# PlakarLabs/plakar

Hardware: AMD Instinct MI355X
Metric: GiB/s chunked (device-resident, cut-points out) at 1/2/4/8 MI355X (higher is better)
Workload: dtype u8; 1 GPU; C1: 1x 1 GiB uniform random buffer per GPU (BASELINE configs[1]); bytes_per_gpu=1073741824, global_bytes=1073741824, buffers_per_gpu=1, chunk_params=FASTCDC min 65536 / normal 1048576 / max 4194304, gear=placeholder (v0.0.8 table unavailable; see DESIGN.md), parallelism=independent buffers, 1 rank per GPU x 1, no collective, streams=2

## Files before the change

plakar_amd/csrc/cdc_kernels.hip:

```cpp
#include <hip/hip_ext.h>
#include <hip/hip_runtime.h>

#include <algorithm>
#include <mutex>
#include <type_traits>
#include <vector>

#include "cdc_hostmem.h"
#include "cdc_internal.h"

namespace cdc {

#ifndef CDC_SPIN_SLEEP
#define CDC_SPIN_SLEEP 1
#endif
constexpr int kSpinSleep = CDC_SPIN_SLEEP;

static constexpr uint64_t kNoHit = ~0ull;
static constexpr uint32_t kRawLaneBytes = 512;
static constexpr uint32_t kWarm = 64;

template <int NT, int COPIES = 32>
__device__ __forceinline__ void fill_gear_lds(uint64_t *tab, const uint64_t *gear, uint32_t sh = 0)
{
    static_assert(NT % 64 == 0, "block size");
    constexpr uint32_t kSlots = 256u * COPIES;
    constexpr int kPer = int((kSlots + NT - 1) / NT);
    uint64_t v[kPer];
#pragma unroll
    for (int i = 0; i < kPer; ++i) {
        const uint32_t x = threadIdx.x + uint32_t(i) * NT;
        v[i] = x < kSlots ? gear[x / COPIES] : 0;
    }
#pragma unroll
    for (int i = 0; i < kPer; ++i) {
        const uint32_t x = threadIdx.x + uint32_t(i) * NT;
        if (x < kSlots) tab[x] = v[i] << sh;
    }
}
constexpr uint32_t kWCopies = 8;
constexpr uint32_t kWEntShift = kWCopies == 32 ? 8 : kWCopies == 16 ? 7 : 6;
static_assert(kWCopies == 8 || kWCopies == 16 || kWCopies == 32, "walker table copies");

__device__ __forceinline__ uint64_t lds_gear(const char *tab, uint32_t addr)
{
    return *reinterpret_cast<const uint64_t *>(tab + addr);
}

typedef __attribute__((address_space(3))) const char lds_char;
typedef __attribute__((address_space(1))) const uint64_t g_u64;
typedef __attribute__((address_space(1))) const uint32_t g_u32;
typedef __attribute__((address_space(1))) const uint8_t g_u8;

__device__ __forceinline__ uint64_t lds_gear(const lds_char *tab, uint32_t addr)
{
    return *reinterpret_cast<__attribute__((address_space(3))) const uint64_t *>(tab + addr);
}

template <typename T>
__device__ __forceinline__ T *as_space(uint64_t addr)
{
    return reinterpret_cast<T *>(uintptr_t(addr));
}

__device__ __forceinline__ const lds_char *as_lds(const char *p)
{
    return as_space<const lds_char>(uint32_t(reinterpret_cast<uintptr_t>(p)));
}

__device__ __forceinline__ uint4 gload16(uint64_t a)
{
    const g_u64 *q = as_space<const g_u64>(a);
    const uint64_t x = q[0], y = q[1];
    return make_uint4(uint32_t(x), uint32_t(x >> 32), uint32_t(y), uint32_t(y >> 32));
}

__device__ __forceinline__ uint32_t gear_addr(uint32_t laneoff, uint32_t word, int k)
{
    return __builtin_amdgcn_perm(laneoff, word, 0x0C0C0004u | (uint32_t(k & 3) << 8));
}

template <uint32_t ESH = kWEntShift>
__device__ __forceinline__ uint32_t wgear_addr(uint32_t wlaneoff, uint32_t word, int k)
{
    if constexpr (ESH == 8) return gear_addr(wlaneoff, word, k);
    return (__builtin_amdgcn_ubfe(word, uint32_t(k & 3) * 8u, 8u) << ESH) | wlaneoff;
}

__device__ __forceinline__ uint32_t key_of(uint64_t fp, uint32_t mlo, uint32_t mhi)
{
    return __builtin_amdgcn_bitop3_b32(uint32_t(fp >> 32), mhi, uint32_t(fp) & mlo, 0xEA);
}

__device__ __forceinline__ uint32_t word_of(const uint4 &d, int i)
{
    return i == 0 ? d.x : i == 1 ? d.y : i == 2 ? d.z : d.w;
}

__device__ __forceinline__ uint32_t umin3(uint32_t a, uint32_t b, uint32_t c)
{
    uint32_t r;
    asm("v_min3_u32 %0, %1, %2, %3" : "=v"(r) : "v"(a), "v"(b), "v"(c));
    return r;
}

template <uint32_t ESH = kWEntShift, typename TP>
__device__ __forceinline__ uint32_t roll16_test(const uint4 &d, uint64_t &fp, TP tab,
                                                uint32_t laneoff, uint32_t mlo, uint32_t mhi)
{
    uint32_t acc = 0xFFFFFFFFu;
#pragma unroll
    for (int k = 0; k < 16; ++k) {
        fp = (fp << 1) + lds_gear(tab, wgear_addr<ESH>(laneoff, word_of(d, k >> 2), k));
        acc = min(acc, key_of(fp, mlo, mhi));
    }
    return acc;
}

template <uint32_t ESH = kWEntShift, typename TP>
__device__ __forceinline__ void roll16(const uint4 &d, uint64_t &fp, TP tab,
                                       uint32_t laneoff)
{
#pragma unroll
    for (int k = 0; k < 16; ++k)
        fp = (fp << 1) + lds_gear(tab, wgear_addr<ESH>(laneoff, word_of(d, k >> 2), k));
}

template <uint32_t ESH = kWEntShift, typename TP>
__device__ __forceinline__ uint64_t group_first_hit(const uint4 &d, uint64_t &fp, uint64_t a,
                                                    uint64_t ts, uint64_t te, uint64_t fz,
                                                    TP tab, uint32_t laneoff,
                                                    uint32_t mlo, uint32_t mhi)
{
    uint64_t hit = kNoHit;
#pragma unroll
    for (int k = 0; k < 16; ++k) {
        const uint64_t pos = a + k;
        const uint64_t g = lds_gear(tab, wgear_addr<ESH>(laneoff, word_of(d, k >> 2), k));
        fp = pos < fz ? 0ull : (fp << 1) + g;
        if (hit == kNoHit && pos >= ts && pos < te && pos >= fz && key_of(fp, mlo, mhi) == 0)
            hit = pos;
    }
    return hit;
}


__device__ __forceinline__ uint32_t to_vgpr(uint32_t x)
{
    uint32_t v;
    asm volatile("v_mov_b32 %0, %1" : "=v"(v) : "s"(x));
    return v;
}

constexpr uint32_t kDbgTs = 16;
constexpr uint32_t kDbgGraph = 32;
constexpr uint32_t kTsScan = 0;
constexpr uint32_t kTsRes = kTsScan + 4 * 4096;
constexpr uint32_t kTsClk = kTsRes + 8 * 16384;
constexpr uint32_t kClkRecs = 4096;
constexpr uint32_t kTsClkN = kTsClk + 4 * kClkRecs;
constexpr uint32_t kTsHw = kTsClkN + 1;
constexpr uint32_t kTsAbort = kTsHw + 4096;
constexpr uint32_t kTsSlots = kTsAbort + 4;
constexpr uint32_t kDbgClk = 64;
__device__ uint64_t g_ts[kTsSlots];

__device__ __forceinline__ void dbg_ts(const Batch &B, uint32_t slot, uint64_t v = ~0ull)
{
    if ((B.debug & kDbgTs) && slot < kTsSlots) g_ts[slot] = v == ~0ull ? __builtin_amdgcn_s_memrealtime() : v;
}

constexpr uint32_t kAbortWord = kMaxBufsPerLaunch;
constexpr uint32_t kLimitWord = kMaxBufsPerLaunch + 1;
constexpr uint64_t kSpinLimit = 200000000ull;
enum : uint32_t { kWaitJunction = 2, kWaitPrev, kWaitLook, kWaitLookSlow, kWaitLast };

struct SpinGuard {
    uint64_t t0 = 0, lim = 0;
    __device__ __forceinline__ bool ok(uint32_t *flags, uint32_t kind, uint64_t a, uint64_t b)
    {
        const uint64_t now = __builtin_amdgcn_s_memrealtime();
        if (!t0) {
            t0 = now;
            lim = __hip_atomic_load(flags + kLimitWord, __ATOMIC_RELAXED, __HIP_MEMORY_SCOPE_AGENT);
            if (!lim) lim = kSpinLimit;
            return true;
        }
        if (__hip_atomic_load(flags + kAbortWord, __ATOMIC_RELAXED, __HIP_MEMORY_SCOPE_AGENT)) return false;
        if (now - t0 < lim) return true;
        if ((threadIdx.x & 63u) == 0) {
            __hip_atomic_store(flags + kAbortWord, kind, __ATOMIC_RELAXED, __HIP_MEMORY_SCOPE_AGENT);
            g_ts[kTsAbort] = kind;
            g_ts[kTsAbort + 1] = a;
            g_ts[kTsAbort + 2] = b;
            g_ts[kTsAbort + 3] = now;
        }
        return false;
    }
};


#ifndef CDC_SCAN_WAVES
#define CDC_SCAN_WAVES 12
#endif
constexpr uint32_t kS2Waves = CDC_SCAN_WAVES;
constexpr uint32_t kStage = 64;
constexpr uint32_t kL = kStage / 16;
constexpr uint32_t kGroups = kStage / 16;
constexpr uint32_t kStageBytes = 64u * kStage;
constexpr uint32_t kGearLdsBytes = 256u * 32u * 8u;
constexpr uint32_t kQCap = 64;
constexpr uint32_t kQBytes = kQCap * 12u;
constexpr uint32_t kFlushTabBytes = 256u * 8u;
static_assert(kGearLdsBytes + kS2Waves * (kStageBytes + kQBytes) + kFlushTabBytes + 37128u <= 160u * 1024u,
              "LDS budget: a scan workgroup and a k_resolve workgroup per CU");
constexpr uint32_t kLaneQuant = 256;

template <int N>
__device__ __forceinline__ void wait_vmcnt()
{
    static_assert(N == 0, "vmcnt");
    asm volatile("s_waitcnt vmcnt(0)" ::: "memory");
}

#ifdef CDC_SCAN_DMA_DEFAULT_POLICY
#define DMA_PIECE(i) "global_load_lds_dwordx4 %" #i ", %[base]\n\t"
#else
#define DMA_PIECE(i) "global_load_lds_dwordx4 %" #i ", %[base] nt\n\t"
#endif
#define DMA_NEXT "s_add_u32 m0, m0, 0x400\n\ts_nop 0\n\t"
__device__ __forceinline__ void dma_stage(uint64_t base_in, uint32_t dst_in, const uint32_t (&off)[kL])
{
    static_assert(kL == 4, "four 1-KiB pieces per stage");
    const uint64_t base = (uint64_t(uint32_t(__builtin_amdgcn_readfirstlane(uint32_t(base_in >> 32)))) << 32) |
                          uint32_t(__builtin_amdgcn_readfirstlane(uint32_t(base_in)));
    const uint32_t dst = __builtin_amdgcn_readfirstlane(dst_in);
    uint32_t keep;
    asm volatile("s_nop 4\n\ts_mov_b32 %[keep], m0\n\ts_mov_b32 m0, %[dst]\n\ts_nop 0\n\t"
                 DMA_PIECE(1) DMA_NEXT DMA_PIECE(2) DMA_NEXT DMA_PIECE(3) DMA_NEXT DMA_PIECE(4)
                 "s_mov_b32 m0, %[keep]\n\ts_nop 1"
                 : [keep] "=&s"(keep)
                 : "v"(off[0]), "v"(off[1]), "v"(off[2]), "v"(off[3]), [base] "s"(base), [dst] "s"(dst)
                 : "memory", "scc");
}

#ifdef CDC_SCAN_DMA_DEFAULT_POLICY
#define DMA_PIECE_IMM(i, o) "global_load_lds_dwordx4 %" #i ", %[base] offset:" #o "\n\t"
#else
#define DMA_PIECE_IMM(i, o) "global_load_lds_dwordx4 %" #i ", %[base] offset:" #o " nt\n\t"
#endif
__device__ __forceinline__ void dma_stage_imm(uint64_t base_in, uint32_t dst_in, const uint32_t (&offi)[kL])
{
    static_assert(kL == 4, "four 1-KiB pieces per stage");
    const uint64_t base = (uint64_t(uint32_t(__builtin_amdgcn_readfirstlane(uint32_t(base_in >> 32)))) << 32) |
                          uint32_t(__builtin_amdgcn_readfirstlane(uint32_t(base_in)));
    const uint32_t dst = __builtin_amdgcn_readfirstlane(dst_in);
    uint32_t keep;
    asm volatile("s_nop 4\n\ts_mov_b32 %[keep], m0\n\ts_mov_b32 m0, %[dst]\n\ts_nop 0\n\t"
                 DMA_PIECE_IMM(1, 0) DMA_PIECE_IMM(2, 1024) DMA_PIECE_IMM(3, 2048) DMA_PIECE_IMM(4, 3072)
                 "s_mov_b32 m0, %[keep]\n\ts_nop 1"
                 : [keep] "=&s"(keep)
                 : "v"(offi[0]), "v"(offi[1]), "v"(offi[2]), "v"(offi[3]), [base] "s"(base), [dst] "s"(dst)
                 : "memory");
}

__device__ __forceinline__ uint32_t wave_ticket(uint32_t *p)
{
    const uint32_t old = __hip_atomic_fetch_add(p, (threadIdx.x & 63u) == 0u ? 1u : 0u, __ATOMIC_RELAXED,
                                                __HIP_MEMORY_SCOPE_AGENT);
    return __builtin_amdgcn_readfirstlane(old);
}

__device__ __forceinline__ uint32_t scan_wave_max(uint32_t v)
{
#pragma unroll
    for (int o = 32; o; o >>= 1) v = max(v, uint32_t(__shfl_xor(int(v), o)));
    return __builtin_amdgcn_readfirstlane(v);
}

__device__ __forceinline__ uint32_t rec_cnt(uint64_t rec) { return uint32_t(rec & ((1u << kRecCntBits) - 1)); }
__device__ __forceinline__ uint32_t rec_ent(uint64_t rec, uint32_t e)
{
    return uint32_t(rec >> (kRecCntBits + kRecEntBits * e)) & ((1u << kRecEntBits) - 1);
}

__device__ __forceinline__ void record_hit(uint64_t &rec, int32_t r)
{
    const uint32_t c = rec_cnt(rec);
    if (c < kRunCap) rec |= uint64_t(uint32_t(r)) << (kRecCntBits + kRecEntBits * c);
    if (c < (1u << kRecCntBits) - 1) ++rec;
}

constexpr uint64_t kMaskLSpill = 16;

__device__ bool maskl_needed(const Batch &B, const DevParams &P, const Workspace &W, const BufDesc &D, uint64_t t,
                             uint32_t lane)
{
    const uint64_t sl = B.scan_lane, tb = 64ull * sl;
    const uint64_t start = t * tb, end = min(D.len, start + tb);
    const uint64_t ra = start / sl, rb = (end - 1) / sl;
    const uint64_t gap = P.normal_size - P.min_size - (P.win - 1);
    const uint32_t kc = uint32_t(gap / sl > 2 ? gap / sl - 1 : 1);
    const uint64_t r_lo = ra > kc + kMaskLSpill ? ra - kc - kMaskLSpill : 0;
    const uint64_t *runs = W.runs + 64ull * D.task_base;
    uint32_t cur = 0;
    for (uint64_t r4 = r_lo; r4 <= rb; r4 += 256) {
        uint64_t rec[4];
#pragma unroll
        for (int j = 0; j < 4; ++j) {
            const uint64_t q = r4 + 64u * j + lane;
            rec[j] = q <= rb ? runs[q] : 1ull;
        }
#pragma unroll
        for (int j = 0; j < 4; ++j) {
            const uint64_t r0 = r4 + 64u * j;
            if (r0 > rb) break;
            const uint64_t E = __ballot(rec_cnt(rec[j]) == 0);
            const uint32_t n = uint32_t(min(rb + 1 - r0, uint64_t(64)));
            const uint64_t Z = ~E & (n == 64 ? ~0ull : (1ull << n) - 1);
            const uint64_t below = Z & ((1ull << lane) - 1);
            const uint32_t prev = below ? lane - 1u - (63u - uint32_t(__builtin_clzll(below))) : cur + lane;
            const uint64_t r = r0 + lane;
            bool need = false;
            if (lane < n) {
                if ((E >> lane) & 1ull)
                    need = r >= ra && prev + 1 >= kc;
                else
                    need = prev >= kc && r + kMaskLSpill >= ra;
            }
            if (__ballot(need)) return true;
            cur = Z ? n - 1u - (63u - uint32_t(__builtin_clzll(Z))) : cur + n;
        }
    }
    return false;
}

template <bool kMaskL, bool kFused>
__device__ __forceinline__ void scan_task(const Batch &B, const DevParams &P, const Workspace &W, char *s_lds,
                                          const char *tab, uint32_t task, uint32_t lane, uint32_t wave,
                                          uint32_t laneoff);

template <bool kMaskL, bool kFused = false>
__device__ __forceinline__ void scan_body(const Batch &B, const DevParams &P, const Workspace &W)
{
    static_assert(!(kMaskL && kFused), "k_scan_f builds both indexes, from the MaskS records' side");
    __shared__ __attribute__((aligned(16)))
    char s_lds[kGearLdsBytes + kS2Waves * (kStageBytes + kQBytes) + (kFused ? kFlushTabBytes : 0u)];
    const uint32_t lane = threadIdx.x & 63u;
    const uint32_t wave = __builtin_amdgcn_readfirstlane(threadIdx.x >> 6);
    const uint32_t laneoff = (lane & 31u) << 3;
    const uint32_t task = blockIdx.x * kS2Waves + wave;
    bool act = true;
    if constexpr (kMaskL) {
        act = false;
        if (task < B.total_tasks) {
            uint32_t bb = 0;
            while (bb + 1 < B.nbufs && task >= B.b[bb + 1].task_base) ++bb;
            const BufDesc &Db = B.b[bb];
            const uint64_t t = task - Db.task_base;
            if (t * 64ull * B.scan_lane < Db.len) act = maskl_needed(B, P, W, Db, t, lane);
            if (lane == 0) W.validL[task] = act ? 1u : 0u;
        }
        if (!__syncthreads_or(act ? 1 : 0)) return;
        if (threadIdx.x == 0 && B.maskl_hint)
            __hip_atomic_store(B.maskl_hint, 1u, __ATOMIC_RELAXED, __HIP_MEMORY_SCOPE_SYSTEM);
    }
    if constexpr (!kMaskL) {
        const uint32_t gt = blockIdx.x * blockDim.x + threadIdx.x, nth = gridDim.x * blockDim.x;
        for (uint32_t i = gt; i < B.total_segs; i += nth) {
            W.xg[i] = 0ull;
            W.sg[i] = 0ull;
        }
        if (gt < kMaxBufsPerLaunch + 4)
            W.flags[gt] = gt == kLimitWord ? uint32_t(B.spin_ticks ? B.spin_ticks : kSpinLimit) : 0u;
        if (gt < 2) W.tick[gt] = 0u;
        if (gt < B.nbufs) B.b[gt].res->status = kRowPending;
        if (threadIdx.x == 0) dbg_ts(B, kTsScan + 4 * blockIdx.x);
    }
    uint32_t clk = 0;
    if (!kMaskL && (B.debug & kDbgClk) && blockIdx.x == 0 && threadIdx.x == 0) {
        clk = kTsClk + 4u * uint32_t(atomicAdd(reinterpret_cast<unsigned long long *>(&g_ts[kTsClkN]), 1ull) % kClkRecs);
        g_ts[clk] = __builtin_amdgcn_s_memrealtime();
        g_ts[clk + 1] = __builtin_amdgcn_s_memtime();
    }
    fill_gear_lds<kS2Waves * 64>(reinterpret_cast<uint64_t *>(s_lds), W.gear,
                                 kFused ? P.fm_sh : kMaskL ? P.fl_sh : P.fs_sh);
    if constexpr (kFused) {
        static_assert(kS2Waves * 64 >= 256, "one entry per thread");
        if (threadIdx.x < 256)
            reinterpret_cast<uint64_t *>(s_lds + kGearLdsBytes + kS2Waves * (kStageBytes + kQBytes))[threadIdx.x] =
                W.gear[threadIdx.x] << P.fs_sh;
    }
    __syncthreads();
    if (!kMaskL && threadIdx.x == 0) {
        dbg_ts(B, kTsScan + 4 * blockIdx.x + 1);
        if (blockIdx.x < 4096)
            dbg_ts(B, kTsHw + blockIdx.x,
                   uint64_t(__builtin_amdgcn_s_getreg(20 | (0 << 6) | (15 << 11))) << 32 |
                       uint32_t(__builtin_amdgcn_s_getreg(4 | (0 << 6) | (31 << 11))));
    }
    const char *tab = s_lds;
    if (!act) return;
    const bool persist = !kMaskL && B.persist != 0;
    auto next_task = [&]() { return wave_ticket(W.tick + 2); };
    for (uint32_t cur = persist ? next_task() : task;;) {
        if (cur >= B.total_tasks) break;
        scan_task<kMaskL, kFused>(B, P, W, s_lds, tab, cur, lane, wave, laneoff);
        if (!persist) break;
        cur = next_task();
    }
    if (clk && threadIdx.x == 0) {
        g_ts[clk + 2] = __builtin_amdgcn_s_memrealtime();
        g_ts[clk + 3] = __builtin_amdgcn_s_memtime();
    }
}

template <bool kMaskL, bool kFused>
__device__ __forceinline__ void scan_task(const Batch &B, const DevParams &P, const Workspace &W, char *s_lds,
                                          const char *tab, uint32_t task, uint32_t lane, uint32_t wave,
                                          uint32_t laneoff)
{
    uint32_t b = 0;
    while (b + 1 < B.nbufs && task >= B.b[b + 1].task_base) ++b;
    const BufDesc &D = B.b[b];

    const uint64_t sl = B.scan_lane;
    const uint64_t ub = reinterpret_cast<uint64_t>(D.data);
    const uint64_t lo_ok = ub & ~15ull, hi_ok = (ub + D.len + 15) & ~15ull;
    const uint64_t seg0 = uint64_t(task - D.task_base) * 64u;
    if (seg0 * sl >= D.len) return;
    const int64_t s = int64_t((seg0 + lane) * sl);
    constexpr uint32_t kLead = 128u;
    const uint32_t T = uint32_t((sl + kLead + (ub & 15u) + kStage - 1u) / kStage);
    const uint64_t wb = ((ub + seg0 * sl) & ~15ull) - kLead;
    const uint64_t base = wb > lo_ok ? wb : lo_ok;
    const uint64_t limw = hi_ok - 16u - base;
    const uint32_t lim = limw > 0x7FFFFFFFull ? 0x7FFFFFFFu : uint32_t(limw);
    const uint32_t ring = uint32_t(reinterpret_cast<uintptr_t>(s_lds)) + kGearLdsBytes + wave * kStageBytes;
    static_assert(kStage == 64 && kL == 4, "pair staging: 64-B stages, one slot");
    const uint32_t half = lane >> 5;
    const uint32_t row = lane & 31u, swz = (row >> 1) & 7u;
    uint32_t offi[4];
    uint32_t om = 0;
#pragma unroll
    for (uint32_t j = 0; j < 4; ++j) {
        const uint32_t r = 8u * j + lane / 8u;
        const uint32_t k = (lane % 8u) ^ ((r >> 1) & 7u);
        const uint32_t o = uint32_t((((ub + (seg0 + r) * sl) & ~15ull) - kLead + 16u * k) - base);
        om = max(om, o);
        offi[j] = o - 1024u * j;
    }
    const uint64_t om0 = scan_wave_max(om);
    const uint64_t half_step = 32ull * sl;
    auto issue = [&](auto PC, uint32_t u, auto FC) {
        constexpr uint32_t Q = decltype(PC)::value;
        constexpr bool kFast = decltype(FC)::value;
        const uint64_t adv = uint64_t(kStage) * (u - Q) + (Q ? half_step : 0ull);
#ifdef CDC_DIAG_NO_DMA
        return;
#endif
        if (kFast || om0 + adv <= uint64_t(lim)) {
#ifdef CDC_DIAG_L2
            dma_stage_imm(lo_ok + ((base + adv - lo_ok) & 0x7FFF0ull), ring, offi);
#else
            dma_stage_imm(base + adv, ring, offi);
#endif
        } else {
            uint32_t eff[4];
#pragma unroll
            for (uint32_t j = 0; j < 4; ++j) eff[j] = min(offi[j] + 1024u * j + uint32_t(adv), lim);
            dma_stage(base, ring, eff);
        }
    };
    const char *rowp = s_lds + kGearLdsBytes + wave * kStageBytes + row * 128u;
    auto load_row = [&](uint4 (&first)[4], uint4 (&second)[4]) {
#ifdef CDC_DIAG_NO_ROW
        asm volatile("" : "+v"(first[0].x), "+v"(second[0].x));
        return;
#endif
#pragma unroll
        for (uint32_t g = 0; g < 4; ++g) first[g] = *reinterpret_cast<const uint4 *>(rowp + 16u * (g ^ swz));
#pragma unroll
        for (uint32_t g = 0; g < 4; ++g) second[g] = *reinterpret_cast<const uint4 *>(rowp + 16u * ((g + 4) ^ swz));
    };
    const uint32_t TT = T + 1;
    const int32_t lag = int32_t(kStage * half);
    const uint32_t vhi = to_vgpr(kFused ? P.fm_mi : kMaskL ? P.fl_hi : P.fs_hi);
    const uint32_t xlo = kMaskL ? P.fl_lo : P.fs_lo, xhi = kMaskL ? P.fl_hi : P.fs_hi;
    const int64_t rel0 = int64_t(((ub + uint64_t(s)) & ~15ull) - kLead) - int64_t(ub);
    using C0 = std::integral_constant<uint32_t, 0>;
    using C1 = std::integral_constant<uint32_t, 1>;
    using Gen = std::integral_constant<bool, false>;
    using Steady = std::integral_constant<bool, true>;

    uint4 A[4] = {}, Bv[4] = {};
#ifdef CDC_DIAG_WAITS
    uint64_t wsum = 0;
    uint32_t nrc = 0;
    const uint64_t tk0 = __builtin_amdgcn_s_memtime();
    const uint64_t rt0 = __builtin_amdgcn_s_memrealtime();
#endif
    static_assert(kLead >= 2 * kStage, "stage 0 must be pure warm-up for both halves");
    issue(C0{}, 0, Gen{});
    wait_vmcnt<0>();
    if (half == 0) load_row(A, Bv);
    asm volatile("s_waitcnt lgkmcnt(0)" ::: "memory");
    if (1 < TT) issue(C1{}, 1, Gen{});
    if (1 < TT) {
        wait_vmcnt<0>();
        if (half == 1) load_row(Bv, A);
        asm volatile("s_waitcnt lgkmcnt(0)" ::: "memory");
        if (2 < TT) issue(C0{}, 2, Gen{});
    }
    uint64_t gv[2][16];
#pragma unroll
    for (int k = 0; k < 16; ++k) gv[0][k] = lds_gear(tab, gear_addr(laneoff, word_of(Bv[0], k >> 2), k));
    uint64_t fp = 0;
    uint64_t rec = 0;
    uint64_t recL = 0;
    const int32_t rr0 = int32_t(rel0 - s) - lag;
    uint64_t *const qf = reinterpret_cast<uint64_t *>(s_lds + kGearLdsBytes + kS2Waves * kStageBytes + wave * kQBytes);
    uint32_t *const qm = reinterpret_cast<uint32_t *>(qf + kQCap);
    static_assert(kQCap == 64, "one flush pass: item j in lane j");
    uint32_t qn = 0;
    const char *const ftab = s_lds + kGearLdsBytes + kS2Waves * (kStageBytes + kQBytes);
    auto rgear = [&](const uint4 &d, int k) -> uint64_t {
        if constexpr (kFused)
            return lds_gear(ftab, __builtin_amdgcn_ubfe(word_of(d, k >> 2), uint32_t(k & 3) * 8u, 8u) << 3);
        else
            return lds_gear(tab, gear_addr(laneoff, word_of(d, k >> 2), k));
    };
    auto flush = [&]() {
        {
            const bool v = lane < qn;
            const uint32_t meta = qm[v ? lane : 0u];
            const uint32_t owner = meta >> 24;
            const int32_t r0 = int32_t(meta & 0xFFFFFFu) - 256;
            const int64_t so = int64_t((seg0 + owner) * sl);
            const int32_t ln = so < int64_t(D.len) ? int32_t(min(int64_t(sl), int64_t(D.len) - so)) : 0;
            const uint64_t a = ub + uint64_t(so + r0);
            auto clamp16 = [&](uint64_t x) { return min(max(x, lo_ok), hi_ok - 16u); };
            const uint4 d0 = gload16(clamp16(a)), d1 = gload16(clamp16(a + 16u));
            uint64_t f = 0;
            if constexpr (kFused) {
                uint4 dw[4];
#pragma unroll
                for (int h = 0; h < 4; ++h) dw[h] = gload16(clamp16(a - 64u + 16u * uint32_t(h)));
#pragma unroll
                for (int k = 0; k < 64; ++k) f = (f << 1) + rgear(dw[k >> 4], k & 15);
            } else {
                f = qf[v ? lane : 0u];
            }
            uint32_t miss = 0, missL = 0;
#pragma unroll
            for (int k = 0; k < 32; ++k) {
                f = (f << 1) + rgear(k < 16 ? d0 : d1, k & 15);
                miss |= min(key_of(f, xlo, xhi), 1u) << k;
                if constexpr (kFused) missL |= min(key_of(f, P.fm_llo, P.fm_lhi), 1u) << k;
            }
            const int32_t lo = r0 < 0 ? -r0 : 0, hi = ln - r0;
            uint32_t vm = lo >= 32 ? 0u : (0xFFFFFFFFu << lo);
            vm &= hi >= 32 ? 0xFFFFFFFFu : (hi <= 0 ? 0u : (1u << hi) - 1u);
            const uint32_t hm = v ? ~miss & vm : 0u;
            const uint32_t hmL = kFused && v ? ~missL & vm : 0u;
            uint64_t todo = __ballot(hm != 0 || hmL != 0);
            while (todo) {
                const int i = int(__builtin_ctzll(todo));
                todo &= todo - 1;
                const uint32_t o = uint32_t(__builtin_amdgcn_readlane(int(owner), i));
                const int32_t ri = __builtin_amdgcn_readlane(r0, i);
                uint32_t m = uint32_t(__builtin_amdgcn_readlane(int(hm), i));
                uint32_t mL = kFused ? uint32_t(__builtin_amdgcn_readlane(int(hmL), i)) : 0u;
                if (lane == o) {
                    for (; m; m &= m - 1) record_hit(rec, ri + int32_t(__builtin_ctz(m)));
                    if constexpr (kFused)
                        for (; mL; mL &= mL - 1) record_hit(recL, ri + int32_t(__builtin_ctz(mL)));
                }
            }
        }
        qn = 0;
    };
    uint64_t f0 = 0;
    uint32_t acc = 0xFFFFFFFFu;
    auto stage = [&](auto PC, auto SC, uint32_t t, uint4 (&cur_d)[4], uint4 (&nxt_d)[4]) {
        constexpr uint32_t Q = decltype(PC)::value;
        constexpr bool kSteady = decltype(SC)::value;
#pragma unroll
        for (uint32_t gi = 0; gi < kGroups; ++gi) {
            if (gi + 1 == kGroups && (kSteady || t + 1 < TT)) {
#ifdef CDC_DIAG_WAITS
                const uint64_t w0 = __builtin_amdgcn_s_memtime();
                wait_vmcnt<0>();
                wsum += __builtin_amdgcn_s_memtime() - w0;
#else
                wait_vmcnt<0>();
#endif
                if (half != Q) load_row(nxt_d, cur_d);
                asm volatile("" ::: "memory");
            }
            const uint4 nx = gi + 1 < kGroups ? cur_d[gi + 1] : nxt_d[0];
            uint64_t (&cg)[16] = gv[gi & 1];
            uint64_t (&ng)[16] = gv[(gi + 1) & 1];
            if ((gi & 1) == 0) {
                f0 = fp;
                acc = 0xFFFFFFFFu;
            }
#pragma unroll
            for (int q = 0; q < 4; ++q) {
#pragma unroll
                for (int k = 4 * q; k < 4 * q + 4; k += 2) {
                    const uint32_t a0 = gear_addr(laneoff, word_of(nx, k >> 2), k);
                    fp = (fp << 1) + cg[k];
                    ng[k] = lds_gear(tab, a0);
                    const uint32_t k0 = uint32_t(fp >> 32) & vhi;
                    const uint32_t a1 = gear_addr(laneoff, word_of(nx, (k + 1) >> 2), k + 1);
                    fp = (fp << 1) + cg[k + 1];
                    ng[k + 1] = lds_gear(tab, a1);
                    acc = umin3(acc, k0, uint32_t(fp >> 32) & vhi);
                    __builtin_amdgcn_sched_barrier(0);
                }
                __builtin_amdgcn_sched_barrier(0);
                if (q == 1 && gi + 1 == kGroups && (kSteady || t + 2 < TT)) {
                    asm volatile("s_waitcnt lgkmcnt(8)" ::: "memory");
                    issue(PC, t + 2, SC);
                    __builtin_amdgcn_sched_barrier(0);
                }
            }
            if (gi & 1) {
#ifndef CDC_DIAG_NO_RECHECK
                const uint64_t fm = __ballot(acc == 0);
#ifdef CDC_DIAG_WAITS
                nrc += fm ? 1u : 0u;
#endif
                if (fm) [[unlikely]] {
                    const uint32_t nq = uint32_t(__popcll(fm));
                    if (qn + nq > kQCap) flush();
                    if (acc == 0) {
                        const uint32_t idx =
                            qn + __builtin_amdgcn_mbcnt_hi(uint32_t(fm >> 32), __builtin_amdgcn_mbcnt_lo(uint32_t(fm), 0u));
                        const int32_t r0 = rr0 + int32_t(kStage * t + 16u * (gi - 1));
                        if constexpr (!kFused) qf[idx] = f0;
                        qm[idx] = uint32_t(r0 + 256) | (lane << 24);
                    }
                    qn += nq;
                }
#else
                rec += acc == 0 ? 1u : 0u;
#endif
            }
        }
    };
    if (1 < TT) stage(C1{}, Gen{}, 1, Bv, A);
    const int64_t room = int64_t(lim) - int64_t(om0) - int64_t(half_step);
    const int64_t tf = room >= 128 ? room / 64 - 1 : 0;
    const uint32_t t_steady = uint32_t(max<int64_t>(2, min<int64_t>(int64_t(TT) - 3, tf)));
    uint32_t t = 2;
    for (; t < t_steady; t += 2) {
        stage(C0{}, Steady{}, t, A, Bv);
        stage(C1{}, Steady{}, t + 1, Bv, A);
    }
    for (; t < TT; t += 2) {
        stage(C0{}, Gen{}, t, A, Bv);
        if (t + 1 < TT) stage(C1{}, Gen{}, t + 1, Bv, A);
    }
    if (qn) flush();
    if (s < int64_t(D.len)) (kMaskL ? W.runsL : W.runs)[64ull * D.task_base + seg0 + lane] = rec;
    if constexpr (kFused) {
        if (s < int64_t(D.len)) W.runsL[64ull * D.task_base + seg0 + lane] = recL;
        if (lane == 0) W.validL[task] = 1u;
    }
    if (!kMaskL && lane == 0) dbg_ts(B, kTsScan + 4 * blockIdx.x + 2 + (wave & 1));
#ifdef CDC_DIAG_WAITS
    if (lane == 0 && 8 * task + 7 < 8 * 16384) {
        uint64_t *o = g_ts + kTsRes + 8 * task;
        o[0] = wsum;
        o[1] = __builtin_amdgcn_s_memtime() - tk0;
        o[2] = rt0;
        o[3] = __builtin_amdgcn_s_memrealtime();
        o[4] = __builtin_amdgcn_s_getreg(4 | (0 << 6) | (31 << 11));
        o[5] = __builtin_amdgcn_s_getreg(20 | (0 << 6) | (15 << 11));
        o[6] = nrc;
        o[7] = wave;
    }
#endif
}

#ifndef CDC_SCAN_LB
#define CDC_SCAN_LB (kS2Waves * 64)
#endif
__global__ __launch_bounds__(CDC_SCAN_LB) void k_scan(const Batch B, const DevParams P, const Workspace W)
{
    scan_body<false>(B, P, W);
}

__global__ __launch_bounds__(kS2Waves * 64) void k_scan_l(const Batch B, const DevParams P, const Workspace W)
{
    scan_body<true>(B, P, W);
}

__global__ __launch_bounds__(CDC_SCAN_LB) void k_scan_f(const Batch B, const DevParams P, const Workspace W)
{
    scan_body<false, true>(B, P, W);
}

constexpr uint32_t kProbeWaves = 4;

__global__ __launch_bounds__(kProbeWaves * 64) void k_maskl_probe(const Batch B, const DevParams P, const Workspace W)
{
    const uint32_t lane = threadIdx.x & 63u;
    const uint32_t task = blockIdx.x * kProbeWaves + __builtin_amdgcn_readfirstlane(threadIdx.x >> 6);
    if (task >= B.total_tasks) return;
    uint32_t b = 0;
    while (b + 1 < B.nbufs && task >= B.b[b + 1].task_base) ++b;
    const BufDesc &D = B.b[b];
    const uint64_t t = task - D.task_base;
    if (t * 64ull * B.scan_lane >= D.len) return;
    if (maskl_needed(B, P, W, D, t, lane) && lane == 0 && B.maskl_hint)
        __hip_atomic_store(B.maskl_hint, 1u, __ATOMIC_RELAXED, __HIP_MEMORY_SCOPE_SYSTEM);
}

constexpr int kDppRowShr = 0x110;

template <int N>
__device__ __forceinline__ uint64_t dpp_shr64_zero(uint64_t v)
{
    const uint32_t lo = __builtin_amdgcn_update_dpp(0u, uint32_t(v), kDppRowShr + N, 0xF, 0xF, true);
    const uint32_t hi = __builtin_amdgcn_update_dpp(0u, uint32_t(v >> 32), kDppRowShr + N, 0xF, 0xF, true);
    return (uint64_t(hi) << 32) | lo;
}

template <int N>
__device__ __forceinline__ uint32_t dpp_shr32_keep(uint32_t v)
{
    return __builtin_amdgcn_update_dpp(v, v, kDppRowShr + N, 0xF, 0xF, false);
}

__device__ __forceinline__ uint64_t readlane64(uint64_t v, int l)
{
    const uint32_t lo = uint32_t(__builtin_amdgcn_readlane(uint32_t(v), l));
    const uint32_t hi = uint32_t(__builtin_amdgcn_readlane(uint32_t(v >> 32), l));
    return (uint64_t(hi) << 32) | lo;
}

__device__ __forceinline__ uint32_t wave_min_u32(uint32_t x)
{
    x = min(x, dpp_shr32_keep<1>(x));
    x = min(x, dpp_shr32_keep<2>(x));
    x = min(x, dpp_shr32_keep<4>(x));
    x = min(x, dpp_shr32_keep<8>(x));
    const uint32_t r0 = uint32_t(__builtin_amdgcn_readlane(x, 15));
    const uint32_t r1 = uint32_t(__builtin_amdgcn_readlane(x, 31));
    const uint32_t r2 = uint32_t(__builtin_amdgcn_readlane(x, 47));
    const uint32_t r3 = uint32_t(__builtin_amdgcn_readlane(x, 63));
    return min(min(r0, r1), min(r2, r3));
}

__global__ __launch_bounds__(64) void k_selftest_wave(const uint64_t *in, uint32_t *out)
{
    __shared__ uint64_t s_in[64];
    __shared__ uint64_t s_v[64];
    const uint32_t j = threadIdx.x;
    uint64_t g = in[j];
    s_in[j] = g;
    uint64_t v = g;
    v += dpp_shr64_zero<1>(v) << 1;
    v += dpp_shr64_zero<2>(v) << 2;
    v += dpp_shr64_zero<4>(v) << 4;
    v += dpp_shr64_zero<8>(v) << 8;
    s_v[j] = v;
    {
        const uint64_t f15 = readlane64(v, 15);
        const uint64_t f31 = readlane64(v, 31) + (f15 << 16);
        const uint64_t f47 = readlane64(v, 47) + (f31 << 16);
        const uint32_t row = j >> 4;
        const uint64_t carry = row == 0 ? 0ull : row == 1 ? f15 : row == 2 ? f31 : f47;
        v += carry << ((j & 15u) + 1u);
    }
    __syncthreads();
    uint64_t ref = 0;
    for (uint32_t k = 0; k <= j; ++k) ref = (ref << 1) + s_in[k];
    uint64_t rowref = 0;
    for (uint32_t k = j & ~15u; k <= j; ++k) rowref = (rowref << 1) + s_in[k];
    const uint32_t bad = ref != v ? 1u : 0u;
    const uint32_t badrow = rowref != s_v[j] ? 1u : 0u;
    auto xv = [&](uint32_t k) { return k >= 40 ? 0xFFFFFFFFu : (uint32_t(s_in[k] >> 32) | 0x80000000u); };
    const uint32_t m = wave_min_u32(xv(j));
    uint32_t mref = 0xFFFFFFFFu;
    for (uint32_t k = 0; k < 64; ++k) mref = min(mref, xv(k));
    const uint32_t mnone = wave_min_u32(j == 63 ? 0x7FFFFFFFu : 0xFFFFFFFFu);
    const uint32_t ba = uint32_t(g), bbv = uint32_t(g >> 32), bc = uint32_t(g >> 16);
    const uint32_t b3bad = __builtin_amdgcn_bitop3_b32(ba, bbv, bc, 0xEA) != ((ba & bbv) | bc) ? 1u : 0u;
    const uint64_t bb = __ballot(bad | (b3bad << 1)), br = __ballot(badrow);
    if (j == 0) {
        out[0] = uint32_t(__popcll(bb));
        out[1] = (m != mref ? 1u : 0u) | (mnone != 0x7FFFFFFFu ? 2u : 0u);
        out[2] = uint32_t(__popcll(br));
        out[3] = uint32_t(br);
        out[4] = m;
        out[5] = mref;
    }
}


struct WalkCtx {
    uint64_t ub;
    uint64_t len;
    uint32_t final_;
    const g_u64 *runs;
    uint64_t sl;
    double inv_sl;
    const lds_char *tab;
    uint32_t laneoff;
    uint32_t lane;
    const uint64_t *gear;
    const g_u64 *runsL;
    const g_u32 *validL;
    uint32_t *flags;
};

__device__ __forceinline__ uint64_t ld_run(const g_u64 *runs, uint64_t q) { return runs[q]; }


template <uint32_t ESH>
__device__ uint64_t raw_scan(const WalkCtx &C, const lds_char *tab, uint32_t laneoff, uint64_t lo, uint64_t hi,
                             uint64_t fz, uint32_t mlo, uint32_t mhi)
{
    const uint64_t H = C.ub + hi, FZ = C.ub + fz;
    uint64_t x = C.ub + lo;
    const uint64_t lb = min<uint64_t>(kRawLaneBytes, max<uint64_t>(64, ((hi - lo + 63) / 64 + 15) & ~15ull));
    while (x < H) {
        const uint64_t A = x & ~15ull;
        const uint64_t bend = min(A + 64ull * lb, H);
        const uint64_t ts = max(x, A + uint64_t(C.lane) * lb);
        const uint64_t te = min(bend, A + uint64_t(C.lane + 1) * lb);
        uint64_t hit = kNoHit;
        if (ts < te) {
            const uint64_t hs = ts >= FZ + kWarm ? ts - kWarm : FZ;
            uint64_t fp = 0;
            for (uint64_t a = hs & ~15ull; a < te; a += 16) {
                const uint4 d = gload16(a);
                if (a >= FZ && a >= ts && a + 16 <= te) {
                    const uint64_t fp0 = fp;
                    if (roll16_test<ESH>(d, fp, tab, laneoff, mlo, mhi) == 0) {
                        uint64_t f = fp0;
                        hit = group_first_hit<ESH>(d, f, a, ts, te, FZ, tab, laneoff, mlo, mhi);
                        break;
                    }
                } else if (a >= FZ && a + 16 <= ts) {
                    roll16<ESH>(d, fp, tab, laneoff);
                } else {
                    hit = group_first_hit<ESH>(d, fp, a, ts, te, FZ, tab, laneoff, mlo, mhi);
                    if (hit != kNoHit) break;
                }
            }
        }
        const uint64_t m = __ballot(hit != kNoHit);
        if (m) return readlane64(hit, __ffsll((unsigned long long)m) - 1) - C.ub;
        x = bend;
    }
    return kNoHit;
}

__device__ __forceinline__ uint64_t raw_first_hit(const WalkCtx &C, uint64_t lo, uint64_t hi, uint64_t fz,
                                               uint32_t mlo, uint32_t mhi)
{
    return raw_scan<kWEntShift>(C, C.tab, C.laneoff, lo, hi, fz, mlo, mhi);
}

__device__ uint64_t trunc_first_hit(const WalkCtx &C, const DevParams &P, uint64_t fz,
                                    uint64_t norm_end, uint64_t lim, uint32_t byte)
{
    const uint32_t j = C.lane;
    const uint64_t pos = fz + j;
    const bool valid = (j + 1 < P.win) && pos < lim;
    uint64_t v = valid ? lds_gear(C.tab, (byte << kWEntShift) | C.laneoff) : 0ull;
    v += dpp_shr64_zero<1>(v) << 1;
    v += dpp_shr64_zero<2>(v) << 2;
    v += dpp_shr64_zero<4>(v) << 4;
    v += dpp_shr64_zero<8>(v) << 8;
    {
        const uint64_t f15 = readlane64(v, 15);
        const uint64_t f31 = readlane64(v, 31) + (f15 << 16);
        const uint64_t f47 = readlane64(v, 47) + (f31 << 16);
        const uint32_t row = j >> 4;
        const uint64_t carry = row == 0 ? 0ull : row == 1 ? f15 : row == 2 ? f31 : f47;
        v += carry << ((j & 15u) + 1u);
    }
    const bool small = pos < norm_end;
    const uint32_t mlo = small ? P.ms_lo : P.ml_lo, mhi = small ? P.ms_hi : P.ml_hi;
    const uint64_t m = __ballot(valid && key_of(v, mlo, mhi) == 0);
    return m ? fz + uint64_t(__ffsll((unsigned long long)m) - 1) : kNoHit;
}

__device__ __forceinline__ uint64_t run_of(const WalkCtx &C, uint64_t x)
{
    uint64_t q = uint64_t(double(x) * C.inv_sl);
    if (q * C.sl > x) --q;
    else if ((q + 1) * C.sl <= x) ++q;
    return q;
}

__device__ __forceinline__ uint64_t rec_first(uint64_t rec, uint64_t rs, uint64_t a, uint64_t b)
{
    const uint32_t n = min(rec_cnt(rec), kRunCap);
    uint64_t best = kNoHit;
#pragma unroll
    for (int i = int(kRunCap) - 1; i >= 0; --i) {
        const uint64_t pos = rs + rec_ent(rec, uint32_t(i));
        if (uint32_t(i) < n && pos >= a && pos < b) best = pos;
    }
    return best;
}

__device__ uint64_t recs_first(const WalkCtx &C, const DevParams &P, uint64_t r0, bool in, uint64_t rec, uint64_t a,
                               uint64_t b, uint64_t fz, bool &done, bool maskl = false)
{
    const uint64_t rs = (r0 + C.lane) * C.sl;
    const uint64_t cand = in ? rec_first(rec, rs, a, b) : kNoHit;
    uint64_t mc = __ballot(cand != kNoHit);
    uint64_t md = __ballot(in && cand == kNoHit && rec_cnt(rec) > kRunCap);
    done = true;
    while (mc | md) {
        const int lf = mc ? __ffsll((unsigned long long)mc) - 1 : 64;
        const int ld = md ? __ffsll((unsigned long long)md) - 1 : 64;
        if (lf < ld) return readlane64(cand, lf);
        const uint64_t rr = r0 + uint64_t(ld);
        const uint64_t lo = max(a, rr * C.sl), hi = min(b, (rr + 1) * C.sl);
        const uint64_t h = raw_first_hit(C, lo, hi, fz, maskl ? P.ml_lo : P.ms_lo, maskl ? P.ml_hi : P.ms_hi);
        if (h != kNoHit) return h;
        md &= ~(1ull << ld);
    }
    done = false;
    return kNoHit;
}

__device__ __forceinline__ uint64_t index_first_hit(const WalkCtx &C, const DevParams &P, uint64_t a, uint64_t b,
                                                 uint64_t fz)
{
    const uint64_t rl = run_of(C, b - 1);
    for (uint64_t r0 = run_of(C, a); r0 <= rl; r0 += 64) {
        const bool in = r0 + C.lane <= rl;
        const uint64_t rec = in ? ld_run(C.runs, r0 + C.lane) : 0ull;
        bool done;
        const uint64_t h = recs_first(C, P, r0, in, rec, a, b, fz, done);
        if (done) return h;
    }
    return kNoHit;
}

__device__ __forceinline__ uint64_t maskl_first_hit(const WalkCtx &C, const DevParams &P, uint64_t a, uint64_t b,
                                                 uint64_t fz)
{
    if (!C.runsL) return raw_first_hit(C, a, b, fz, P.ml_lo, P.ml_hi);
    const uint64_t ra = run_of(C, a), rl = run_of(C, b - 1);
    for (uint64_t r0 = ra & ~63ull; r0 <= rl; r0 += 64) {
        const uint64_t lo = max(a, r0 * C.sl), hi = min(b, (r0 + 64) * C.sl);
        if (C.validL[r0 >> 6]) {
            const bool in = r0 + C.lane >= ra && r0 + C.lane <= rl;
            const uint64_t rec = in ? ld_run(C.runsL, r0 + C.lane) : 0ull;
            bool done;
// ... 1203 lines not shown
```

Before: 5031 GiB/s.

## Drop stored fingerprint from recheck queue, recompute with warmup; parametrize scan roll

The hit queue no longer stores the 64-bit rolling fingerprint. The flush pass instead reloads the 64 preceding bytes and recomputes the fingerprint. This shrinks per-wave queue LDS and removes the f0 bookkeeping from the hot loop. The scan inner loop is regrouped into configurable roll chunks with optional scheduling group barriers, and a filter-group size knob is added. Steady-state DMA issue now uses an incrementing pointer instead of recomputing offsets. The trade-off is extra global loads and gear lookups on every flush.

```diff
diff --git a/plakar_amd/csrc/cdc_kernels.hip b/plakar_amd/csrc/cdc_kernels.hip
--- a/plakar_amd/csrc/cdc_kernels.hip
+++ b/plakar_amd/csrc/cdc_kernels.hip
@@ -209,8 +209,25 @@
 constexpr uint32_t kGroups = kStage / 16;
 constexpr uint32_t kStageBytes = 64u * kStage;
 constexpr uint32_t kGearLdsBytes = 256u * 32u * 8u;
+#ifndef CDC_SCAN_FILTER_GROUPS
+#define CDC_SCAN_FILTER_GROUPS 2
+#endif
+constexpr uint32_t kFilt = CDC_SCAN_FILTER_GROUPS;
+static_assert((kFilt == 2 || kFilt == 4) && kGroups % kFilt == 0, "a filter group is half a stage or a whole one");
+#ifndef CDC_SCAN_ROLL_BYTES
+#define CDC_SCAN_ROLL_BYTES 2
+#endif
+#ifndef CDC_SCAN_GROUP_SCHED
+#define CDC_SCAN_GROUP_SCHED 0
+#endif
+constexpr int kRoll = CDC_SCAN_ROLL_BYTES;
+static_assert(kRoll == 2 || kRoll == 4 || kRoll == 8, "regions tile the 8 bytes before the DMA issue");
+#ifndef CDC_SCAN_FLUSH_BATCH
+#define CDC_SCAN_FLUSH_BATCH (4 + CDC_SCAN_FILTER_GROUPS)
+#endif
+constexpr uint32_t kFlushBatch = CDC_SCAN_FLUSH_BATCH;
 constexpr uint32_t kQCap = 64;
-constexpr uint32_t kQBytes = kQCap * 12u;
+constexpr uint32_t kQBytes = kQCap * 4u;
 constexpr uint32_t kFlushTabBytes = 256u * 8u;
 static_assert(kGearLdsBytes + kS2Waves * (kStageBytes + kQBytes) + kFlushTabBytes + 37128u <= 160u * 1024u,
               "LDS budget: a scan workgroup and a k_resolve workgroup per CU");
@@ -452,13 +469,20 @@
     }
     const uint64_t om0 = scan_wave_max(om);
     const uint64_t half_step = 32ull * sl;
+    uint64_t pb = base;
     auto issue = [&](auto PC, uint32_t u, auto FC) {
         constexpr uint32_t Q = decltype(PC)::value;
         constexpr bool kFast = decltype(FC)::value;
-        const uint64_t adv = uint64_t(kStage) * (u - Q) + (Q ? half_step : 0ull);
 #ifdef CDC_DIAG_NO_DMA
         return;
 #endif
+#ifndef CDC_DIAG_L2
+        if constexpr (kFast) {
+            dma_stage_imm(Q ? pb + half_step : pb, ring, offi);
+            return;
+        }
+#endif
+        const uint64_t adv = uint64_t(kStage) * (u - Q) + (Q ? half_step : 0ull);
         if (kFast || om0 + adv <= uint64_t(lim)) {
 #ifdef CDC_DIAG_L2
             dma_stage_imm(lo_ok + ((base + adv - lo_ok) & 0x7FFF0ull), ring, offi);
@@ -519,8 +543,7 @@
     uint64_t rec = 0;
     uint64_t recL = 0;
     const int32_t rr0 = int32_t(rel0 - s) - lag;
-    uint64_t *const qf = reinterpret_cast<uint64_t *>(s_lds + kGearLdsBytes + kS2Waves * kStageBytes + wave * kQBytes);
-    uint32_t *const qm = reinterpret_cast<uint32_t *>(qf + kQCap);
+    uint32_t *const qm = reinterpret_cast<uint32_t *>(s_lds + kGearLdsBytes + kS2Waves * kStageBytes + wave * kQBytes);
     static_assert(kQCap == 64, "one flush pass: item j in lane j");
     uint32_t qn = 0;
     const char *const ftab = s_lds + kGearLdsBytes + kS2Waves * (kStageBytes + kQBytes);
@@ -530,6 +553,8 @@
         else
             return lds_gear(tab, gear_addr(laneoff, word_of(d, k >> 2), k));
     };
+    constexpr int kFB = 16 * int(kFilt);
+    using mask_t = std::conditional_t<kFilt == 4, uint64_t, uint32_t>;
     auto flush = [&]() {
         {
             const bool v = lane < qn;
@@ -540,47 +565,58 @@
             const int32_t ln = so < int64_t(D.len) ? int32_t(min(int64_t(sl), int64_t(D.len) - so)) : 0;
             const uint64_t a = ub + uint64_t(so + r0);
             auto clamp16 = [&](uint64_t x) { return min(max(x, lo_ok), hi_ok - 16u); };
-            const uint4 d0 = gload16(clamp16(a)), d1 = gload16(clamp16(a + 16u));
             uint64_t f = 0;
-            if constexpr (kFused) {
-                uint4 dw[4];
-#pragma unroll
-                for (int h = 0; h < 4; ++h) dw[h] = gload16(clamp16(a - 64u + 16u * uint32_t(h)));
-#pragma unroll
-                for (int k = 0; k < 64; ++k) f = (f << 1) + rgear(dw[k >> 4], k & 15);
-            } else {
-                f = qf[v ? lane : 0u];
-            }
-            uint32_t miss = 0, missL = 0;
-#pragma unroll
-            for (int k = 0; k < 32; ++k) {
-                f = (f << 1) + rgear(k < 16 ? d0 : d1, k & 15);
-                miss |= min(key_of(f, xlo, xhi), 1u) << k;
-                if constexpr (kFused) missL |= min(key_of(f, P.fm_llo, P.fm_lhi), 1u) << k;
+            mask_t miss = 0, missL = 0;
+            static_assert((4 + kFilt) % kFlushBatch == 0, "whole batches");
+#pragma unroll 1
+            for (uint32_t h0 = 0; h0 < 4 + kFilt; h0 += kFlushBatch) {
+                uint4 d[kFlushBatch];
+#pragma unroll
+                for (uint32_t i = 0; i < kFlushBatch; ++i) d[i] = gload16(clamp16(a - 64u + 16u * (h0 + i)));
+#pragma unroll
+                for (uint32_t i = 0; i < kFlushBatch; ++i) {
+                    uint32_t ms = 0, msL = 0;
+#pragma unroll
+                    for (int k = 0; k < 16; ++k) {
+                        f = (f << 1) + rgear(d[i], k);
+                        ms |= min(key_of(f, xlo, xhi), 1u) << k;
+                        if constexpr (kFused) msL |= min(key_of(f, P.fm_llo, P.fm_lhi), 1u) << k;
+                    }
+                    if (h0 + i >= 4) {
+                        miss |= mask_t(ms) << (16u * (h0 + i - 4));
+                        if constexpr (kFused) missL |= mask_t(msL) << (16u * (h0 + i - 4));
+                    }
+                }
             }
             const int32_t lo = r0 < 0 ? -r0 : 0, hi = ln - r0;
-            uint32_t vm = lo >= 32 ? 0u : (0xFFFFFFFFu << lo);
-            vm &= hi >= 32 ? 0xFFFFFFFFu : (hi <= 0 ? 0u : (1u << hi) - 1u);
-            const uint32_t hm = v ? ~miss & vm : 0u;
-            const uint32_t hmL = kFused && v ? ~missL & vm : 0u;
+            mask_t vm = lo >= kFB ? mask_t(0) : mask_t(~mask_t(0) << lo);
+            vm &= hi >= kFB ? ~mask_t(0) : (hi <= 0 ? mask_t(0) : mask_t((mask_t(1) << hi) - 1u));
+            const mask_t hm = v ? ~miss & vm : mask_t(0);
+            const mask_t hmL = kFused && v ? ~missL & vm : mask_t(0);
             uint64_t todo = __ballot(hm != 0 || hmL != 0);
+            auto lane_mask = [](mask_t x, int i) -> mask_t {
+                const uint32_t l = uint32_t(__builtin_amdgcn_readlane(int(uint32_t(x)), i));
+                if constexpr (sizeof(mask_t) == 8)
+                    return mask_t(uint64_t(uint32_t(__builtin_amdgcn_readlane(int(uint32_t(uint64_t(x) >> 32)), i))) << 32 | l);
+                else
+                    return l;
+            };
             while (todo) {
                 const int i = int(__builtin_ctzll(todo));
                 todo &= todo - 1;
                 const uint32_t o = uint32_t(__builtin_amdgcn_readlane(int(owner), i));
                 const int32_t ri = __builtin_amdgcn_readlane(r0, i);
-                uint32_t m = uint32_t(__builtin_amdgcn_readlane(int(hm), i));
-                uint32_t mL = kFused ? uint32_t(__builtin_amdgcn_readlane(int(hmL), i)) : 0u;
+                mask_t m = lane_mask(hm, i);
+                mask_t mL = kFused ? lane_mask(hmL, i) : mask_t(0);
                 if (lane == o) {
-                    for (; m; m &= m - 1) record_hit(rec, ri + int32_t(__builtin_ctz(m)));
+                    for (; m; m &= m - 1) record_hit(rec, ri + int32_t(__builtin_ctzll(m)));
                     if constexpr (kFused)
-                        for (; mL; mL &= mL - 1) record_hit(recL, ri + int32_t(__builtin_ctz(mL)));
+                        for (; mL; mL &= mL - 1) record_hit(recL, ri + int32_t(__builtin_ctzll(mL)));
                 }
             }
         }
         qn = 0;
     };
-    uint64_t f0 = 0;
     uint32_t acc = 0xFFFFFFFFu;
     auto stage = [&](auto PC, auto SC, uint32_t t, uint4 (&cur_d)[4], uint4 (&nxt_d)[4]) {
         constexpr uint32_t Q = decltype(PC)::value;
@@ -601,32 +637,31 @@
             const uint4 nx = gi + 1 < kGroups ? cur_d[gi + 1] : nxt_d[0];
             uint64_t (&cg)[16] = gv[gi & 1];
             uint64_t (&ng)[16] = gv[(gi + 1) & 1];
-            if ((gi & 1) == 0) {
-                f0 = fp;
-                acc = 0xFFFFFFFFu;
-            }
-#pragma unroll
-            for (int q = 0; q < 4; ++q) {
-#pragma unroll
-                for (int k = 4 * q; k < 4 * q + 4; k += 2) {
+            if (gi % kFilt == 0) acc = 0xFFFFFFFFu;
+#pragma unroll
+            for (int c = 0; c < 16; c += kRoll) {
+                uint32_t key[kRoll];
+#pragma unroll
+                for (int k = c; k < c + kRoll; ++k) {
                     const uint32_t a0 = gear_addr(laneoff, word_of(nx, k >> 2), k);
                     fp = (fp << 1) + cg[k];
                     ng[k] = lds_gear(tab, a0);
-                    const uint32_t k0 = uint32_t(fp >> 32) & vhi;
-                    const uint32_t a1 = gear_addr(laneoff, word_of(nx, (k + 1) >> 2), k + 1);
-                    fp = (fp << 1) + cg[k + 1];
-                    ng[k + 1] = lds_gear(tab, a1);
-                    acc = umin3(acc, k0, uint32_t(fp >> 32) & vhi);
-                    __builtin_amdgcn_sched_barrier(0);
+                    key[k - c] = uint32_t(fp >> 32) & vhi;
+                    if (k & 1) acc = umin3(acc, key[k - c - 1], key[k - c]);
                 }
+#if CDC_SCAN_GROUP_SCHED
+                __builtin_amdgcn_sched_group_barrier(0x002, kRoll, 0);
+                __builtin_amdgcn_sched_group_barrier(0x100, kRoll, 0);
+                __builtin_amdgcn_sched_group_barrier(0x002, 2 * kRoll + kRoll / 2, 0);
+#endif
                 __builtin_amdgcn_sched_barrier(0);
-                if (q == 1 && gi + 1 == kGroups && (kSteady || t + 2 < TT)) {
+                if (c + kRoll == 8 && gi + 1 == kGroups && (kSteady || t + 2 < TT)) {
                     asm volatile("s_waitcnt lgkmcnt(8)" ::: "memory");
                     issue(PC, t + 2, SC);
                     __builtin_amdgcn_sched_barrier(0);
                 }
             }
-            if (gi & 1) {
+            if (gi % kFilt == kFilt - 1) {
 #ifndef CDC_DIAG_NO_RECHECK
                 const uint64_t fm = __ballot(acc == 0);
 #ifdef CDC_DIAG_WAITS
@@ -638,8 +673,8 @@
                     if (acc == 0) {
                         const uint32_t idx =
                             qn + __builtin_amdgcn_mbcnt_hi(uint32_t(fm >> 32), __builtin_amdgcn_mbcnt_lo(uint32_t(fm), 0u));
-                        const int32_t r0 = rr0 + int32_t(kStage * t + 16u * (gi - 1));
-                        if constexpr (!kFused) qf[idx] = f0;
+                        const uint32_t st = kSteady ? uint32_t(pb) - uint32_t(base) - (2u - Q) * kStage : kStage * t;
+                        const int32_t r0 = rr0 + int32_t(st + 16u * (gi + 1 - kFilt));
                         qm[idx] = uint32_t(r0 + 256) | (lane << 24);
                     }
                     qn += nq;
@@ -655,7 +690,8 @@
     const int64_t tf = room >= 128 ? room / 64 - 1 : 0;
     const uint32_t t_steady = uint32_t(max<int64_t>(2, min<int64_t>(int64_t(TT) - 3, tf)));
     uint32_t t = 2;
-    for (; t < t_steady; t += 2) {
+    pb = base + uint64_t(kStage) * (t + 2);
+    for (; t < t_steady; t += 2, pb += 2 * kStage) {
         stage(C0{}, Steady{}, t, A, Bv);
         stage(C1{}, Steady{}, t + 1, Bv, A);
     }
```

Result: no change. 5020 GiB/s (-0.2%).
